# kupc25648/MOP-truss-MARL

Hardware: AMD Instinct MI355X
Metric: env steps/sec (batched FEM solves) at 4096 envs (higher is better)
Workload: dtype f64; 1 GPU; synthetic random-geometry 2-row trusses, 32 nodes / 80 elements / 60 DOF, FEM-only env.step (action decode + FP64 assembly/solve + stresses + point), no agent; envs_per_gpu=4096, global_envs=4096, nodes=32, elements=80, ndof=60, half_bandwidth=7, lanes_per_env=16, rows_per_lane=1, parallelism=env-batch sharded over 1 GPU(s), no data-path collective

## Files before the change

mop-truss-marl_amd/csrc/truss_body.h:

```cpp
#pragma once
#include <stdint.h>
#include <math.h>

#ifndef TB_SCHED_FENCE
#define TB_SCHED_FENCE()
#endif
#ifndef TRUSS_HD
#error "define TRUSS_HD (e.g. __device__ __forceinline__) before including truss_body.h"
#endif

#define TF_TOP 1
#define TF_RESX 2
#define TF_RESY 4
#define TF_LOAD_BRIDGE 8
#define TF_LOAD_ROOF 16

#define TB_NO_DECODE 0x1u
#define TB_CLAMP_INPLACE 0x2u
#define TB_EMIT_OBS 0x4u

#if defined(__clang__)
typedef uint32_t tb_u4 __attribute__((ext_vector_type(4)));
typedef uint32_t tb_u2 __attribute__((ext_vector_type(2)));
typedef float tb_f4 __attribute__((ext_vector_type(4)));
// ... 554 lines not shown
    }
  }

  TRUSS_HD void phase_assemble_nodes(const TopoDev &T) {
    const double *EV = evsh(T);
    const int16_t *AD = t_adj8(T), *DO = t_diagoff(T);
    double *K = kb(T);
    static_assert(NDEG == 8, "adjacency rows are read as one 16-byte unit");
    tb_u4 adj[NPL];
    int dof[NPL][3];
    double cc[NPL], cs[NPL], ss[NPL];
#pragma unroll
    for (int i = 0; i < NPL; ++i) {
      const int n0 = g + G * i, n = n0 < T.N ? n0 : T.N - 1;
      adj[i] = *(const tb_u4 *)(AD + n * NDEG);
      dof[i][0] = DO[3 * n];
      dof[i][1] = DO[3 * n + 1];
      dof[i][2] = DO[3 * n + 2];
      cc[i] = cs[i] = ss[i] = 0.0;
    }
#pragma unroll
    for (int h = 0; h < 2; ++h) {
      double ev[NPL][4][3];
#pragma unroll
      for (int i = 0; i < NPL; ++i)
#pragma unroll
        for (int a = 0; a < 4; ++a) {
          const uint32_t w = adj[i][2 * h + (a >> 1)];
          const int e = (a & 1) ? (int)(w >> 16) : (int)(w & 0xffffu);
          ev[i][a][0] = EV[3 * e + 0];
          ev[i][a][1] = EV[3 * e + 1];
          ev[i][a][2] = EV[3 * e + 2];
        }
#pragma unroll
      for (int i = 0; i < NPL; ++i)
#pragma unroll
        for (int a = 0; a < 4; ++a) {
          cc[i] += ev[i][a][0];
          cs[i] += ev[i][a][1];
          ss[i] += ev[i][a][2];
        }
    }
#pragma unroll
    for (int i = 0; i < NPL; ++i) {
      K[dof[i][0]] = cc[i];
      K[dof[i][1]] = ss[i];
      K[dof[i][2]] = cs[i];
    }
    for (int n = g + G * NPL; n < T.N; n += G) {
      double c2 = 0.0, s2 = 0.0, x2 = 0.0;
#pragma unroll
      for (int a = 0; a < NDEG; ++a) {
        const int e = AD[n * NDEG + a];
        c2 += EV[3 * e + 0];
        x2 += EV[3 * e + 1];
        s2 += EV[3 * e + 2];
      }
      K[DO[3 * n]] = c2;
      K[DO[3 * n + 1]] = s2;
      K[DO[3 * n + 2]] = x2;
    }
    const int idA = T.nteams == 1 ? T.ndof : T.ndof - T.KA;
    for (int r = idA + g; r < T.rowsA; r += G) K[r * W + r % W] = 1.0;
    for (int r = T.KA + T.mid + g; r < T.rowsB; r += G) K[(T.rowsA + r) * W + r % W] = 1.0;
  }

  TRUSS_HD void solver_scratch_init(const TopoDev &T) {
    double *Z = zs(T);
    const uint8_t *ZC = t_zcode(T);
    const int lbit = is_roof ? 4 : 2;
    {
      const int zt = T.zlen * T.nteams;
      constexpr int ZIT = 6;
#pragma unroll
      for (int i = 0; i < ZIT; ++i) {
        const int r0 = g + G * i, r = r0 < zt ? r0 : zt - 1;
        const int c = ZC[r];
        Z[r] = (c & lbit) ? ((c & 1) ? load_y : load_x) : 0.0;
      }
      for (int r = g + G * ZIT; r < zt; r += G) {
        const int c = ZC[r];
        Z[r] = (c & lbit) ? ((c & 1) ? load_y : load_x) : 0.0;
      }
    }
    tb_d2 *X2 = (tb_d2 *)__builtin_assume_aligned(xsol(T), 16);
    const tb_d2 z2 = {0.0, 0.0};
    for (int r = g; r < (T.zslot + 2) / 2; r += G) X2[r] = z2;
    double *RB = rbuf(T);
    for (int i = g; i < T.n_rest; i += G) RB[i] = 0.0;
  }

  TRUSS_HD void solver_init(const TopoDev &T) {
#pragma unroll
    for (int s = 0; s < RPL; ++s) {
      int r = gs + WL * s;
#pragma unroll
      for (int c = 0; c < W; ++c) R[s][c] = (c <= r) ? Kt[r * W + c] : Kt[c * W + r];
      rhs[s] = Zt[r];
    }
#pragma unroll
    for (int j = 0; j < W; ++j) xs[j] = 0.0;
  }

  double zkeep[RPL];
  TRUSS_HD void pivot_write(const TopoDev &T, int k, int kk) {
#pragma unroll
    for (int s = 0; s < RPL; ++s) Kt[k * W + gs + WL * s] = R[s][kk];
    bx = rhs[kk / WL];
  }
  TRUSS_HD void factor_z_store(const TopoDev &T, int kb, int c, int cnt) {
#pragma unroll
    for (int s = 0; s < RPL; ++s) {
      const int off = (gs + WL * s - c + W) % W;
      double *zp = off < cnt ? Zt + kb + off : ZRt + gs;
      *zp = zkeep[s];
    }
  }

  TRUSS_HD void pivot_update(const TopoDev &T, int k, int kk) {
    double col[W];
    {
      const double *Kn = Kt + (k + W) * W;
#pragma unroll
      for (int s = 0; s < RPL; ++s) ecol[s] = Kn[gs + WL * s];
    }
#pragma unroll
    for (int i = 0; i < W / 2; ++i) {
      tb_d2 v = ((const tb_d2 *)__builtin_assume_aligned(Kt + k * W, 16))[i];
      col[2 * i] = v[0];
      col[2 * i + 1] = v[1];
    }
    const double zk = tb_team_bcast(*this, kk % WL);
    if (gs == kk % WL) zkeep[kk / WL] = bx;
    const double d = col[kk];
    const double inv = tb_rcp(d);
#pragma unroll
    for (int s = 0; s < RPL; ++s) {
      double l = R[s][kk] * inv;
#pragma unroll
      for (int j = 0; j < W; ++j)
        if (j != kk) R[s][j] = fma(-l, col[j], R[s][j]);
      rhs[s] = fma(-l, zk, rhs[s]);
    }
#pragma unroll
    for (int s = 0; s < RPL; ++s) R[s][kk] = ecol[s];
    if (gs == kk % WL) {
      const int sp = kk / WL;
#pragma unroll
      for (int j = 0; j < W; ++j)
        if (j != kk) R[sp][j] = fr[sp][j];
      rhs[sp] = frhs[sp];
    }
  }
  double fr[RPL][W], frhs[RPL], ecol[RPL];
  TRUSS_HD void factor_rows_fetch(const TopoDev &T, int kb) {
#pragma unroll
    for (int s = 0; s < RPL; ++s) {
      const int rn = kb + W + gs + WL * s;
      const tb_d2 *K2 = (const tb_d2 *)__builtin_assume_aligned(Kt + rn * W, 16);
#pragma unroll
      for (int i = 0; i < W / 2; ++i) {
        tb_d2 v = K2[i];
        fr[s][2 * i] = v[0];
        fr[s][2 * i + 1] = v[1];
      }
      frhs[s] = Zt[rn];
    }
  }

  TRUSS_HD void pivot_check(const TopoDev &T) {
    const int lim = (T.nteams == 2 && team == 1) ? T.KA : (T.nteams == 2 ? T.KA + W : T.KA);
    for (int k = gs; k < lim; k += WL) {
      const double d = Kt[k * W + k % W];
      if (!(d > 0.0) || !(d < 1.7e308)) bad = 1;
    }
  }

  TRUSS_HD int win_row(const TopoDev &T, int slot) const { return T.KA + ((slot - T.KA % W + W) % W); }
  TRUSS_HD void merge_post(const TopoDev &T) {
    if (team == 1) {
      double *M = (double *)(L + T.o_mrg);
#pragma unroll
      for (int j = 0; j < W; ++j) M[gs * W + j] = R[0][j];
      M[W * W + gs] = rhs[0];
    }
  }
  TRUSS_HD void merge_take(const TopoDev &T) {
    if (team == 0) {
      const double *M = (const double *)(L + T.o_mrg);
      const int lim = T.ndof - T.KA;
      const int p = win_row(T, gs);
      const int pb = T.ndof - 1 - p;
#pragma unroll
      for (int j = 0; j < W; ++j) {
        const int c = win_row(T, j);
        const int cb = T.ndof - 1 - c;
        const bool ok = p < lim && c < lim;
        const double add = M[ok ? (pb % W) * W + (cb % W) : 0];
        R[0][j] += ok ? add : 0.0;
      }
      const double az = M[W * W + (p < lim ? pb % W : 0)];
      rhs[0] += p < lim ? az : 0.0;
    }
  }

  double bc[RPL][W], bz[RPL], bd[RPL];
  double nc[RPL][W], nz[RPL], nd[RPL];
  double bx;
  double myx[RPL] = {};
  TRUSS_HD void backsub_rows_fetch(const TopoDev &T, int kb) {
#pragma unroll
    for (int s = 0; s < RPL; ++s) {
      const int p = kb + gs + WL * s;
      const int pc = p < 0 ? 0 : p;
      const tb_d2 *K2 = (const tb_d2 *)__builtin_assume_aligned(Kt + pc * W, 16);
#pragma unroll
      for (int i = 0; i < W / 2; ++i) {
        tb_d2 v = K2[i];
        nc[s][2 * i] = v[0];
        nc[s][2 * i + 1] = v[1];
      }
      nz[s] = Zt[pc];
      nd[s] = Kt[pc * W + pc % W];
    }
  }
  TRUSS_HD void backsub_rows_adopt() {
#pragma unroll
    for (int s = 0; s < RPL; ++s) {
#pragma unroll
      for (int j = 0; j < W; ++j) bc[s][j] = nc[s][j];
      bz[s] = nz[s];
      bd[s] = tb_rcp(nd[s]);
    }
  }
  TRUSS_HD void backsub_step(const TopoDev &T, int k, int kk) {
    const int s = kk / WL;
    double acc0 = bz[s], acc1 = 0.0;
#pragma unroll
    for (int m = W - 1; m >= 2; --m) {
      const int j = (kk + m) % W;
      if (m & 1) acc1 = fma(-bc[s][j], xs[j], acc1);
      else acc0 = fma(-bc[s][j], xs[j], acc0);
    }
    const int jn = (kk + 1) % W;
    double acc = fma(-bc[s][jn], xs[jn], acc0 + acc1);
    bx = acc * bd[s];
  }
  TRUSS_HD void backsub_share(int kk) {
    xs[kk] = tb_team_bcast(*this, kk % WL);
    if (gs == kk % WL) myx[kk / WL] = bx;
  }
  TRUSS_HD bool owns_row(const TopoDev &T, int p) const {
    if (T.nteams == 1) return true;
    return team == 0 ? p < T.ndof - T.KA : p < T.KA;
  }
  TRUSS_HD void backsub_flush(const TopoDev &T, int kb) {
    double *XS = xsol(T);
#pragma unroll
    for (int s = 0; s < RPL; ++s) {
      const int p = kb + gs + WL * s;
      XS[owns_row(T, p) ? orig_pos(T, team, p) : T.zslot + 1] = myx[s];
    }
  }
  TRUSS_HD void backsub_flush_mid(const TopoDev &T) {
    double *XS = xsol(T);
    const int p = win_row(T, gs);
    XS[(team == 0 && owns_row(T, p)) ? p : T.zslot + 1] = myx[0];
  }
  TRUSS_HD void backsub_reload(const TopoDev &T) {
    const double *XS = xsol(T);
#pragma unroll
    for (int j = 0; j < W; ++j) {
      const int o = orig_pos(T, team, win_row(T, j));
      xs[j] = XS[(o >= 0 && o < T.ndof) ? o : T.zslot];
    }
  }

  TRUSS_HD float *oq0(const TopoDev &T) { return (float *)(L + T.o_kb + T.so_q0); }
  TRUSS_HD float *osr(const TopoDev &T) { return (float *)(L + T.o_kb + T.so_sr); }
  TRUSS_HD float *odisp(const TopoDev &T) { return (float *)(L + T.o_kb + T.so_disp); }
  TRUSS_HD float *omu(const TopoDev &T) { return (float *)(L + T.o_kb + T.so_mu); }
  TRUSS_HD float *omd(const TopoDev &T) { return (float *)(L + T.o_kb + T.so_md); }
  TRUSS_HD uint8_t *ocomp(const TopoDev &T) { return (uint8_t *)(L + T.o_kb + T.so_comp); }

  TRUSS_HD void phase_post_elements(const TopoDev &T, const StepArgsDev &A) {
    const double *XS = xsol(T);
    const int16_t *EX = t_exs(T);
    float *Q = oq0(T), *SR = osr(T);
    uint8_t *CP = ocomp(T);
    tb_u2 ex[EPL];
    double qv[EPL];
    float srv[EPL];
#pragma unroll
    for (int i = 0; i < EPL; ++i) {
      const int e = g + G * i;
      const int ee = e < T.E ? e : T.E - 1;
      ex[i] = *(const tb_u2 *)(EX + 4 * ee);
    }
    double v[EPL][4];
#pragma unroll
    for (int i = 0; i < EPL; ++i) {
      v[i][0] = XS[ex[i][0] & 0xffffu];
      v[i][1] = XS[ex[i][0] >> 16];
      v[i][2] = XS[ex[i][1] & 0xffffu];
      v[i][3] = XS[ex[i][1] >> 16];
    }
// ... 375 lines not shown
  TRUSS_HD void obs_nodes_raw(const TopoDev &T, const StepArgsDev &A) {
    if constexpr (EMIT) {
      load_params(T);
      float *Lf = (float *)L;
      const float *Y = ysh(T), *X = xsh(T), *TG = tgsh(T), *DS = odisp(T), *MU = omu(T), *MD = omd(T);
      const uint8_t *NFL = t_nflags(T);
      const float maxdef32 = (float)max_def;
      const int lbit = is_roof ? TF_LOAD_ROOF : TF_LOAD_BRIDGE;
#pragma unroll
      for (int c = 0; c < NDYN; ++c) {
        pmn[c] = INFINITY;
        pmx[c] = -INFINITY;
      }
#pragma unroll
      for (int i = 0; i < NPL; ++i) {
        const int n = g + G * i;
        const int nc = n < T.N ? n : T.N - 1;
        const int fl = NFL[nc];
        const float y = Y[nc];
        float *f = nfe[i];
        f[0] = X[nc];
        f[1] = y;
        f[2] = (fl & lbit) ? 1.0f : 0.0f;
        f[3] = MU[nc];
        f[4] = MD[nc];
        f[5] = (fl & TF_TOP) ? TG[nc] / (y + 1e-6f) : 0.0f;
        f[6] = fabsf(DS[2 * nc + 1]);
        const float ratio = f[6] / maxdef32;
        f[7] = fminf(ratio, 1.0f) * (ratio > 1.0f ? 1.0f : 0.5f);
        f[8] = ratio > 1.0f ? 1.0f : 0.0f;
        const tb_f4 raw = {f[2], f[5], f[6], ratio >= 1.0f ? 1.0f : 0.0f};
        ((tb_f4 *)(Lf + T.b_nraw))[nc] = raw;
        if (n < T.N) {
#pragma unroll
          for (int c = 0; c < NDYN; ++c) {
            pmn[c] = fminf(pmn[c], f[c]);
            pmx[c] = fmaxf(pmx[c], f[c]);
          }
        }
      }
    }
  }

  TRUSS_HD void obs_bank_fill(const TopoDev &T, const StepArgsDev &A) {
    if constexpr (EMIT) {
      float *Lf = (float *)L;
      float nv[NPL][NDYN];
#pragma unroll
      for (int c = 0; c < NDYN; ++c) {
        const float lo = tb_group_min(*this, c), hi = tb_group_max(*this, c);
        const float inv = tb_rcpf(hi - lo + 1e-6f);
#pragma unroll
        for (int i = 0; i < NPL; ++i) nv[i][c] = (nfe[i][c] - lo) * inv;
      }
#pragma unroll
      for (int i = 0; i < NPL; ++i) {
        const int n = g + G * i;
        const int nc = n < T.N ? n : T.N - 1;
        const tb_f4 a = {nv[i][0], nv[i][1], nv[i][2], nv[i][3]}, b = {nv[i][4], nv[i][5], nv[i][6], nv[i][7]};
        ((tb_f4 *)(Lf + T.b_nna))[nc] = a;
        ((tb_f4 *)(Lf + T.b_nnb))[nc] = b;
        Lf[T.b_nn8 + nc] = nv[i][8];
      }
    }
  }

  TRUSS_HD tb_f4 gather4(const float *Lf, const tb_u2 t) const {
    const tb_f4 v = {Lf[t[0] & 0xffffu], Lf[t[0] >> 16], Lf[t[1] & 0xffffu], Lf[t[1] >> 16]};
    return v;
  }
  template <int IT>
  TRUSS_HD void emit_rows(float *out, size_t row_floats, int nc, const tb_u2 (&tab)[IT]) const {
    if (!out) return;
    const float *Lf = (const float *)L;
    tb_f4 *o4 = (tb_f4 *)(out + (size_t)env * row_floats);
#pragma unroll
    for (int b0 = 0; b0 < IT; b0 += KB) {
      if (b0 * G < nc) {
        tb_f4 v[KB];
#pragma unroll
        for (int k = 0; k < KB; ++k)
          if (b0 + k < IT) v[k] = gather4(Lf, tab[b0 + k]);
#pragma unroll
        for (int k = 0; k < KB; ++k)
          if (b0 + k < IT) TB_OBS_STORE(&o4[chunk_of(b0 + k, nc)], v[k]);
      }
    }
  }
  TRUSS_HD void obs_nxe_table(const TopoDev &T) {
    if constexpr (EMIT) {
      if (T.nxe_cw != 4) return;
      const tb_u2 *tab = TB_TAB(tb_u2, TB, T.f_tnxe);
#pragma unroll
      for (int i = 0; i < IE; ++i) ete[i] = tab[i * G + g];
    }
  }
  TRUSS_HD void emit_nxe_narrow(const TopoDev &T, const StepArgsDev &A) const {
    if (!A.nxe) return;
    const float *Lf = (const float *)L;
    const uint16_t *tab = TB_TAB(uint16_t, TB, T.f_tnxe);
    float *o = A.nxe + (size_t)env * 21 * T.E;
    const int nc = T.nc_nxe;
    if (T.nxe_cw == 2) {
      for (int q0 = g; q0 < nc; q0 += 4 * G) {
        tb_f2 v[4];
#pragma unroll
        for (int k = 0; k < 4; ++k) {
          const int q = q0 + k * G < nc ? q0 + k * G : nc - 1;
          const tb_f2 w = {Lf[tab[2 * q]], Lf[tab[2 * q + 1]]};
          v[k] = w;
        }
#pragma unroll
        for (int k = 0; k < 4; ++k) {
          const int q = q0 + k * G < nc ? q0 + k * G : nc - 1;
          TB_OBS_STORE((tb_f2 *)o + q, v[k]);
        }
      }
    } else {
      for (int q0 = g; q0 < nc; q0 += 4 * G) {
        float v[4];
#pragma unroll
        for (int k = 0; k < 4; ++k) v[k] = Lf[tab[q0 + k * G < nc ? q0 + k * G : nc - 1]];
#pragma unroll
        for (int k = 0; k < 4; ++k) TB_OBS_STORE(o + (q0 + k * G < nc ? q0 + k * G : nc - 1), v[k]);
      }
    }
  }
  TRUSS_HD void obs_emit_raw_rows(const TopoDev &T, const StepArgsDev &A) {
    if constexpr (EMIT) {
      if (!active) return;
      if (T.nxe_cw == 4) emit_rows<IE>(A.nxe, (size_t)21 * T.E, T.nc_nxe, ete);
      else emit_nxe_narrow(T, A);
      emit_rows<IN_>(A.nxn, (size_t)12 * T.N, T.nc_nxn, etn);
    }
  }
  TRUSS_HD void obs_emit_xn(const TopoDev &T, const StepArgsDev &A) {
    if constexpr (EMIT) {
      if (!active) return;
      emit_rows<IX>(A.x_n, (size_t)13 * T.N, T.nc_xn, etx);
    }
  }
};

#ifndef TRUSS_ST
#define TRUSS_ST(i)
#endif
#define TRUSS_STREAM_SEG1(PH, T, A) PH(obs_emit_as(T, A));
#define TRUSS_STREAM_SEG2(PH, T, A) \
  PH(obs_emit_tc(T, A));            \
  PH(obs_nxe_table(T));
#define TRUSS_STREAM_SEG3(PH, T, A) \
  PH(obs_emit_raw_rows(T, A));      \
  PH(obs_emit_xn(T, A));
#define TRUSS_STEP_SCHEDULE(PH, PH_NS, BAR, T, A)                                   \
  TRUSS_ST(0);                                                                      \
  PH(phase_stage(T, A));                                                            \
  TRUSS_ST(1);                                                                      \
  PH(phase_decode(T, A));                                                           \
  if ((T).n_sym_nodes > 0 && !((A).flags & TB_NO_DECODE)) { PH(phase_sym_nodes(T)); } \
  TRUSS_ST(2);                                                                      \
  PH(phase_sizing(T, A));                                                           \
  if ((T).n_sym_elems > 0 && !((A).flags & TB_NO_DECODE)) { PH(phase_sym_elems(T)); } \
  if (EMIT_) { EMIT_POINT(1); TRUSS_ST(19); }  \
  PH_NS(rollout_prefetch(T, A));  \
  TRUSS_ST(3);                                                                      \
  PH(phase_elements(T, A));                                                         \
  TRUSS_ST(10);                                                                     \
  PH(phase_assemble_nodes(T));                                                      \
  TRUSS_ST(11);                                                                     \
  PH(solver_scratch_init(T));                                                       \
  TRUSS_ST(4);                                                                      \
  PH(solver_init(T));                                                               \
  {                                                                                 \
                                                                                    \
    const int kend_ = (T).nteams == 2 ? (T).KA + W_ : (T).KA;                       \
    int kb_ = 0;                                                                    \
    for (; kb_ + W_ <= (T).KA; kb_ += W_) {                                         \
      PH_NS(factor_rows_fetch(T, kb_));                                             \
      TRUSS_UNROLL                                                                  \
      for (int kk_ = 0; kk_ < W_; ++kk_) {                                          \
        PH(pivot_write(T, kb_ + kk_, kk_));                                         \
        PH_NS(pivot_update(T, kb_ + kk_, kk_));                                     \
      }                                                                             \
      PH_NS(factor_z_store(T, kb_, 0, W_));                                         \
    }                                                                               \
    TRUSS_ST(13);                                                                   \
                                  \
    if ((T).nteams == 2 && W_ <= 8) {                                               \
      const int c0_ = (T).KA % W_;                                                  \
      TRUSS_UNROLL                                                                  \
      for (int c_ = 0; c_ < W_; ++c_) {                                             \
        if (c_ == c0_) {                                                            \
          if (c_ > 0) { PH_NS(factor_rows_fetch(T, kb_)); }                         \
          TRUSS_UNROLL                                                              \
          for (int kk_ = 0; kk_ < c_; ++kk_) {                                      \
            PH(pivot_write(T, kb_ + kk_, kk_));                                     \
            PH_NS(pivot_update(T, kb_ + kk_, kk_));                                 \
          }                                                                         \
          if (c_ > 0) { PH_NS(factor_z_store(T, kb_, 0, c_)); }                     \
          PH(merge_post(T));                                                        \
          PH(merge_take(T));                                                        \
          TRUSS_UNROLL                                                              \
          for (int i_ = 0; i_ < W_; ++i_) {                                         \
            if ((c_ + i_) % W_ == 0) { PH_NS(factor_rows_fetch(T, (T).KA + i_)); }  \
            PH(pivot_write(T, (T).KA + i_, (c_ + i_) % W_));                        \
            PH_NS(pivot_update(T, (T).KA + i_, (c_ + i_) % W_));                    \
          }                                                                         \
          PH_NS(factor_z_store(T, (T).KA, c_, W_));                                 \
        }                                                                           \
      }                                                                             \
    } else if ((T).nteams == 2) {  \
      for (; kb_ < kend_; kb_ += W_) {                                              \
        PH_NS(factor_rows_fetch(T, kb_));                                           \
        TRUSS_UNROLL                                                                \
        for (int kk_ = 0; kk_ < W_; ++kk_) {                                        \
          if (kb_ + kk_ < kend_) {                                                  \
            if (kb_ + kk_ == (T).KA) {                                              \
              PH(merge_post(T));                                                    \
              PH(merge_take(T));                                                    \
            }                                                                       \
            PH(pivot_write(T, kb_ + kk_, kk_));                                     \
            PH_NS(pivot_update(T, kb_ + kk_, kk_));                                 \
          }                                                                         \
        }                                                                           \
        PH_NS(factor_z_store(T, kb_, 0, kend_ - kb_ < W_ ? kend_ - kb_ : W_));      \
      }                                                                             \
    }                                                                               \
    BAR();                                                                          \
    PH_NS(pivot_check(T));                                                          \
    TRUSS_ST(5);                                                                    \
                \
    kb_ = ((kend_ - 1) / W_) * W_;                                                  \
    PH_NS(backsub_rows_fetch(T, kb_));                                              \
    if ((T).nteams == 2 && W_ <= 8) {                                               \
      const int c0_ = (T).KA % W_;                                                  \
      TRUSS_UNROLL                                                                  \
      for (int c_ = 0; c_ < W_; ++c_) {                                             \
        if (c_ == c0_) {                                                            \
          PH_NS(backsub_rows_adopt());                                              \
          PH_NS(backsub_rows_fetch(T, kb_ - W_));                                   \
          TRUSS_UNROLL                                                              \
          for (int i_ = W_ - 1; i_ >= 0; --i_) {                                    \
            PH_NS(backsub_step(T, (T).KA + i_, (c_ + i_) % W_));                    \
            PH_NS(backsub_share((c_ + i_) % W_));                                   \
            if ((c_ + i_) % W_ == 0 && i_ > 0) {         \
              kb_ -= W_;                                                            \
              PH_NS(backsub_rows_adopt());                                          \
              PH_NS(backsub_rows_fetch(T, kb_ - W_));                               \
            }                                                                       \
          }                                                                         \
          PH_NS(backsub_flush_mid(T));                                              \
          BAR();                                                                    \
          PH_NS(backsub_reload(T));                                                 \
          TRUSS_UNROLL                                                              \
          for (int kk_ = c_ - 1; kk_ >= 0; --kk_) {                                 \
            PH_NS(backsub_step(T, kb_ + kk_, kk_));                                 \
            PH_NS(backsub_share(kk_));                                              \
          }                                                                         \
          if (c_ > 0) { PH_NS(backsub_flush(T, kb_)); }                             \
          kb_ -= W_;                                                                \
        }                                                                           \
      }                                                                             \
    } else if ((T).nteams == 2) {                                                   \
      for (; kb_ >= 0 && kb_ + W_ - 1 >= (T).KA - 1; kb_ -= W_) {                   \
        PH_NS(backsub_rows_adopt());                                                \
        PH_NS(backsub_rows_fetch(T, kb_ - W_));                                     \
        TRUSS_UNROLL                                                                \
        for (int kk_ = W_ - 1; kk_ >= 0; --kk_) {                                   \
          if (kb_ + kk_ < kend_) {                                                  \
            if (kb_ + kk_ == (T).KA - 1) {                                          \
              PH_NS(backsub_flush_mid(T));                                          \
              BAR();                                                                \
              PH_NS(backsub_reload(T));                                             \
            }                                                                       \
            PH_NS(backsub_step(T, kb_ + kk_, kk_));                                 \
            PH_NS(backsub_share(kk_));                                              \
          }                                                                         \
        }                                                                           \
        PH_NS(backsub_flush(T, kb_));                                               \
      }                                                                             \
    }                                                                               \
    TRUSS_ST(14);                                                                   \
    for (; kb_ >= 0; kb_ -= W_) {                                                   \
      PH_NS(backsub_rows_adopt());                                                  \
      PH_NS(backsub_rows_fetch(T, kb_ - W_));                                       \
      TRUSS_UNROLL                                                                  \
      for (int kk_ = W_ - 1; kk_ >= 0; --kk_) {                                     \
        PH_NS(backsub_step(T, kb_ + kk_, kk_));                                     \
        PH_NS(backsub_share(kk_));                                                  \
      }                                                                             \
      PH_NS(backsub_flush(T, kb_));                                                 \
    }                                                                               \
  }                                                                                 \
  BAR();                                                                            \
  TRUSS_ST(6);                                                                      \
  PH_NS(rollout_stash(T, A));                                                       \
  PH(phase_post_elements(T, A));                                                    \
  if (EMIT_) {                                                                      \
    EMIT_POINT(2);                                                                  \
    TRUSS_ST(18);                                                                   \
    PH(obs_elements_bank(T, A));                                                    \
  }                                                                                 \
  TRUSS_ST(7);                                                                      \
  PH(phase_post_nodes(T, A));                                                       \
  TRUSS_ST(8);                                                                      \
  if (EMIT_) {   \
    TRUSS_ST(15);                                                                   \
    PH(obs_nodes_raw(T, A));                                                        \
    TRUSS_ST(16);                                                                   \
    PH(obs_bank_fill(T, A));                                                        \
    EMIT_POINT(3);                                                                  \
    TRUSS_ST(17);                                                                   \
  }                                                                                 \
  PH_NS(phase_finish(T, A));                                                        \
  TRUSS_ST(12);                                                                     \
  PH_NS(phase_store(T, A));                                                         \
  TRUSS_ST(9);

struct ObsArgsDev {
  int32_t B;
  uint32_t flags;
  const float *x, *y;
  const int32_t *sec;
  const float *mu, *md, *target, *disp, *q0, *sr;
  const uint8_t *comp;
  const double *env_params;
  float *x_n, *A_s, *A_ts, *A_cs, *nxn, *nxe;
  int32_t tile_rows;
  int32_t n_split;
};

struct ObsLane {
  int lane, env;
  char *L;
  float maxdef32;
  int is_roof;
  int role;
  int minmax_done;

  TRUSS_HD float *raw() { return (float *)L; }
  TRUSS_HD float *mn(const TopoDev &T) { return raw() + T.N * 13; }
  TRUSS_HD float *mx(const TopoDev &T) { return mn(T) + 13; }
  TRUSS_HD float *part(const TopoDev &T) { return mx(T) + 13; }
  TRUSS_HD float *mats(const TopoDev &T) { return (float *)(L + (((size_t)(T.N * 13 + 26 + 128) * 4 + 15) & ~(size_t)15)); }

  TRUSS_HD void init(int lane_, int block, int tile, const TopoDev &, const ObsArgsDev &A, char *lds) {
    lane = lane_;
    env = block;
    L = lds;
    role = A.n_split <= 1 ? 0 : tile == 0 ? 2 : 1;
    minmax_done = 0;
    const double *P = A.env_params + (size_t)env * 8;
    maxdef32 = (float)P[2];
    is_roof = P[7] != 0.0;
  }

  TRUSS_HD void phase_nodes(const TopoDev &T, const ObsArgsDev &A) {
    if (role == 1) return;
    const size_t bn = (size_t)env * T.N;
// ... 182 lines not shown
```

mop-truss-marl_amd/csrc/truss_hip.hip:

```cpp
#include <hip/hip_runtime.h>

#include <atomic>
#include <cstdint>
#include <cstdio>
#include <cstring>
#include <type_traits>

#include "../../include/truss_mi355.h"

#pragma clang fp contract(off)

#define TRUSS_HD __device__ __forceinline__
#define TRUSS_UNROLL _Pragma("unroll")
#define TB_SCHED_FENCE() __builtin_amdgcn_sched_barrier(0)
#define TB_STREAM_STORE(p, v) __builtin_nontemporal_store((v), (p))
#ifdef TRUSS_OBS_STORE_NT
#define TB_OBS_STORE(p, v) __builtin_nontemporal_store((v), (p))
#else
#define TB_OBS_STORE(p, v) (*(p) = (v))
#endif

__device__ __forceinline__ void tb_lds_add(double *p, double v) { unsafeAtomicAdd(p, v); }

template <int WL, int SRC>
__device__ __forceinline__ double tb_dpp_bcast(double v) {
  const int lo = __double2loint(v), hi = __double2hiint(v);
  int rlo, rhi;
  if constexpr (WL == 16) {
    rlo = __builtin_amdgcn_update_dpp(lo, lo, 0x150 + SRC, 0xf, 0xf, false);
    rhi = __builtin_amdgcn_update_dpp(hi, hi, 0x150 + SRC, 0xf, 0xf, false);
  } else if constexpr (WL == 8) {
    rlo = __builtin_amdgcn_update_dpp(lo, lo, 0x150 + SRC, 0xf, 0x3, false);
    rlo = __builtin_amdgcn_update_dpp(rlo, lo, 0x150 + 8 + SRC, 0xf, 0xc, false);
    rhi = __builtin_amdgcn_update_dpp(hi, hi, 0x150 + SRC, 0xf, 0x3, false);
    rhi = __builtin_amdgcn_update_dpp(rhi, hi, 0x150 + 8 + SRC, 0xf, 0xc, false);
  } else {
    static_assert(WL == 4, "team width");
    constexpr int qp = SRC | (SRC << 2) | (SRC << 4) | (SRC << 6);
    rlo = __builtin_amdgcn_update_dpp(lo, lo, qp, 0xf, 0xf, false);
    rhi = __builtin_amdgcn_update_dpp(hi, hi, qp, 0xf, 0xf, false);
  }
  return __hiloint2double(rhi, rlo);
}
template <class LN>
__device__ __forceinline__ double tb_team_bcast(LN &ln, int src) {
  constexpr int WL = LN::WL_;
  switch (src) {
#define TB_CASE(i) \
  case i:          \
    if constexpr (i < WL) return tb_dpp_bcast<WL, i>(ln.bx); else break;
    TB_CASE(0) TB_CASE(1) TB_CASE(2) TB_CASE(3) TB_CASE(4) TB_CASE(5) TB_CASE(6) TB_CASE(7)
    TB_CASE(8) TB_CASE(9) TB_CASE(10) TB_CASE(11) TB_CASE(12) TB_CASE(13) TB_CASE(14) TB_CASE(15)
#undef TB_CASE
  }
  return ln.bx;
}

__device__ __forceinline__ double tb_rcp(double d) {
  double r = __builtin_amdgcn_rcp(d);
  r = fma(fma(-d, r, 1.0), r, r);
  r = fma(fma(-d, r, 1.0), r, r);
  return r;
}

__device__ __forceinline__ float tb_rcpf(float d) {
  float r = __builtin_amdgcn_rcpf(d);
  return fmaf(fmaf(-d, r, 1.0f), r, r);
}

#ifdef TRUSS_STOP_AT
#define TRUSS_ST(i) do { if ((i) == TRUSS_STOP_AT) return; } while (0)
#endif
#ifdef TRUSS_STAMPS
__device__ unsigned long long g_truss_stamps[32];
__device__ unsigned long long g_truss_span[4096][6];
#define TRUSS_ST(i)                                                  \
  do {                                                               \
    __builtin_amdgcn_sched_barrier(0);                               \
    if (threadIdx.x == 0 && blockIdx.x == gridDim.x / 2) g_truss_stamps[i] = clock64(); \
    if (threadIdx.x == 0 && ((i) == 0 || (i) == 9) && blockIdx.x < 4096) {              \
      g_truss_span[blockIdx.x][(i) == 0 ? 0 : 2] = clock64();                            \
      g_truss_span[blockIdx.x][(i) == 0 ? 1 : 3] = wall_clock64();                       \
    }                                                                \
    __builtin_amdgcn_sched_barrier(0);                               \
  } while (0)
#endif

__device__ __forceinline__ double tb_rsqrt(double x) {
  double r = __builtin_amdgcn_rsq(x);
  r = r * fma(-0.5 * x, r * r, 1.5);
  r = r * fma(-0.5 * x, r * r, 1.5);
  return r;
}

template <int G, bool MAX>
__device__ __forceinline__ float tb_group_reduce(float v) {
  auto op = [](float a, float b) { return MAX ? fmaxf(a, b) : fminf(a, b); };
  auto dpp = [](float x, auto ctrl) {
    return __int_as_float(__builtin_amdgcn_update_dpp(0, __float_as_int(x), decltype(ctrl)::value, 0xf, 0xf, false));
  };
  if constexpr (G >= 2) v = op(v, dpp(v, std::integral_constant<int, 0xB1>{}));
  if constexpr (G >= 4) v = op(v, dpp(v, std::integral_constant<int, 0x4E>{}));
  if constexpr (G >= 8) v = op(v, dpp(v, std::integral_constant<int, 0x141>{}));
  if constexpr (G >= 16) v = op(v, dpp(v, std::integral_constant<int, 0x140>{}));
  if constexpr (G >= 32) v = op(v, __shfl_xor(v, 16));
  if constexpr (G >= 64) v = op(v, __shfl_xor(v, 32));
  return v;
}
template <class LN>
__device__ __forceinline__ float tb_group_min(LN &ln, int c) { return tb_group_reduce<LN::G_, false>(ln.pmn[c]); }
template <class LN>
__device__ __forceinline__ float tb_group_max(LN &ln, int c) { return tb_group_reduce<LN::G_, true>(ln.pmx[c]); }

template <int G>
__device__ __forceinline__ double tb_group_reduce_sum(double v) {
  auto dpp = [](double x, auto ctrl) {
    const int lo = __builtin_amdgcn_update_dpp(0, __double2loint(x), decltype(ctrl)::value, 0xf, 0xf, false);
    const int hi = __builtin_amdgcn_update_dpp(0, __double2hiint(x), decltype(ctrl)::value, 0xf, 0xf, false);
    return __hiloint2double(hi, lo);
  };
  if constexpr (G >= 2) v = v + dpp(v, std::integral_constant<int, 0xB1>{});
  if constexpr (G >= 4) v = v + dpp(v, std::integral_constant<int, 0x4E>{});
  if constexpr (G >= 8) v = v + dpp(v, std::integral_constant<int, 0x141>{});
  if constexpr (G >= 16) v = v + dpp(v, std::integral_constant<int, 0x140>{});
  if constexpr (G >= 32) v = v + __shfl_xor(v, 16);
  if constexpr (G >= 64) v = v + __shfl_xor(v, 32);
  return v;
}
template <class LN>
__device__ __forceinline__ double tb_group_sum_d(LN &ln, int which) {
  return tb_group_reduce_sum<LN::G_>(which == 0 ? ln.p_vol : which == 1 ? ln.p_dt : ln.p_en);
}
template <class LN>
__device__ __forceinline__ float tb_group_max_f(LN &ln, int which) {
  return tb_group_reduce<LN::G_, true>(which == 0 ? ln.p_c1 : which == 1 ? ln.p_c2 : (float)ln.bad);
}

template <class LN, class TD>
__device__ __forceinline__ bool tb_obs_timed_out(LN &ln, const TD &T) {
  if constexpr (LN::EMIT_) return *((const __attribute__((address_space(3))) int *)(ln.TB + T.o_flag) + 1) != 0;
  return false;
}

#include "truss_body.h"

typedef __attribute__((address_space(3))) int tb_lds_word;
__device__ __forceinline__ tb_lds_word *tb_flag_ptr(char *lds, int o_flag) { return (tb_lds_word *)(lds + o_flag); }
__device__ __forceinline__ void tb_publish(char *lds, int o_flag, int k) {
  __builtin_amdgcn_wave_barrier();
#ifdef TRUSS_FLAG_RELAXED
  __builtin_amdgcn_fence(__ATOMIC_RELEASE, "wavefront");
  if (threadIdx.x == 0) __hip_atomic_store(tb_flag_ptr(lds, o_flag), k, __ATOMIC_RELAXED, __HIP_MEMORY_SCOPE_WORKGROUP);
#else
  if (threadIdx.x == 0) __hip_atomic_store(tb_flag_ptr(lds, o_flag), k, __ATOMIC_RELEASE, __HIP_MEMORY_SCOPE_WORKGROUP);
#endif
}
#ifndef TB_AWAIT_SPINS
#define TB_AWAIT_SPINS (1 << 22)
#endif
__device__ __forceinline__ bool tb_await(char *lds, int o_flag, int k) {
  for (int spin = 0; spin < TB_AWAIT_SPINS; ++spin) {
    const int v = __hip_atomic_load(tb_flag_ptr(lds, o_flag), __ATOMIC_ACQUIRE, __HIP_MEMORY_SCOPE_WORKGROUP);
    if (__builtin_amdgcn_readfirstlane(v) >= k) return true;
    __builtin_amdgcn_s_sleep(1);
  }
  return false;
}

template <class LN>
__device__ __forceinline__ void tb_obs_timeout(LN &ln, char *lds, int o_flag, int32_t *status) {
  if ((threadIdx.x & 63) == 0) *(tb_flag_ptr(lds, o_flag) + 1) = 1;
  if (ln.g == 0 && ln.active && status) atomicOr(&status[ln.env], TRUSS_STATUS_OBS_TIMEOUT);
}

template <int G, int WL, int RPL, int EPL, bool EMIT>
__global__ __launch_bounds__(EMIT ? 128 : 64) void truss_step_kernel(const TopoDev T, const StepArgsDev A) {
  extern __shared__ __attribute__((aligned(16))) char smem[];
  StepLane<G, WL, RPL, EPL, EMIT> ln;
  ln.init(threadIdx.x & 63, blockIdx.x, T, A, smem);
  constexpr int W_ = StepLane<G, WL, RPL, EPL, EMIT>::W;
  constexpr bool EMIT_ = EMIT;
  if constexpr (EMIT) {
    if (threadIdx.x == 0) {
      *tb_flag_ptr(smem, T.o_flag) = 0;
      *(tb_flag_ptr(smem, T.o_flag) + 1) = 0;
    }
    __syncthreads();
    if (threadIdx.x >= 64) {
#define SPH(call) \
  ln.call;        \
  __builtin_amdgcn_fence(__ATOMIC_RELEASE, "wavefront"); \
  __builtin_amdgcn_wave_barrier();                        \
  __builtin_amdgcn_fence(__ATOMIC_ACQUIRE, "wavefront")
#ifdef TRUSS_STAMPS
#define SST(i)                                                                                        \
  do {                                                                                                \
    __builtin_amdgcn_sched_barrier(0);                                                                \
    if (threadIdx.x == 64 && blockIdx.x == gridDim.x / 2) g_truss_stamps[i] = clock64();              \
    if (threadIdx.x == 64 && ((i) == 20 || (i) == 26) && blockIdx.x < 4096)                           \
      g_truss_span[blockIdx.x][(i) == 20 ? 4 : 5] = wall_clock64();                                   \
    __builtin_amdgcn_sched_barrier(0);                                                                \
  } while (0)
#else
#define SST(i)
#endif
      ln.emit_tables_load(T);
      __builtin_amdgcn_s_waitcnt(0);
      bool ok = tb_await(smem, T.o_flag, 1);
      if (ok) {
        SST(20);
        TRUSS_STREAM_SEG1(SPH, T, A)
        SST(21);
        ok = tb_await(smem, T.o_flag, 2);
      }
      if (ok) {
        SST(22);
        TRUSS_STREAM_SEG2(SPH, T, A)
        SST(23);
        ok = tb_await(smem, T.o_flag, 3);
      }
      if (ok) {
        SST(24);
        TRUSS_STREAM_SEG3(SPH, T, A)
        SST(25);
      } else {
        tb_obs_timeout(ln, smem, T.o_flag, A.status);
      }
#ifdef TRUSS_STAMPS
      __builtin_amdgcn_s_waitcnt(0);
      SST(26);
#endif
#undef SST
#undef SPH
      return;
    }
  }
#define TB_WAVE_SYNC()                                    \
  do {                                                    \
    __builtin_amdgcn_fence(__ATOMIC_RELEASE, "wavefront"); \
    __builtin_amdgcn_wave_barrier();                      \
    __builtin_amdgcn_fence(__ATOMIC_ACQUIRE, "wavefront"); \
  } while (0)
#define PH(call) \
  ln.call;       \
  TB_WAVE_SYNC()
#define PH_NS(call) ln.call
#define BAR() TB_WAVE_SYNC()
#ifdef TRUSS_FAULT_DROP_PUBLISH3
#define EMIT_POINT(k) do { if ((k) != 3) tb_publish(smem, T.o_flag, k); } while (0)
#else
#define EMIT_POINT(k) tb_publish(smem, T.o_flag, k)
#endif
  TRUSS_STEP_SCHEDULE(PH, PH_NS, BAR, T, A)
#undef PH
#undef PH_NS
#undef BAR
#undef EMIT_POINT
#undef TB_WAVE_SYNC
}

struct RolloutDev {
  TopoDev T;
  StepArgsDev A;
  int32_t n_steps, n_sets;
  size_t gstride, tstride;
};
template <int G, int WL, int RPL, int EPL>
__global__ __launch_bounds__(64) void truss_rollout_kernel(const RolloutDev P_) {
  extern __shared__ __attribute__((aligned(16))) char smem[];
  constexpr int W_ = StepLane<G, WL, RPL, EPL, false>::W;
  constexpr bool EMIT_ = false;
#define TB_WAVE_SYNC()                                    \
  do {                                                    \
    __builtin_amdgcn_fence(__ATOMIC_RELEASE, "wavefront"); \
    __builtin_amdgcn_wave_barrier();                      \
    __builtin_amdgcn_fence(__ATOMIC_ACQUIRE, "wavefront"); \
  } while (0)
#define PH(call) \
  ln.call;       \
  TB_WAVE_SYNC()
#define PH_NS(call) ln.call
#define BAR() TB_WAVE_SYNC()
#define EMIT_POINT(k) (void)0
  const int n_steps = P_.n_steps;
  for (int s = 0; s < n_steps; ++s) {
    typedef const char __attribute__((address_space(4))) *tb_kernarg_ptr;
    tb_kernarg_ptr ka = (tb_kernarg_ptr)__builtin_amdgcn_kernarg_segment_ptr();
    asm volatile("" : "+s"(ka));
    const RolloutDev &P = *(const RolloutDev *)ka;
    const TopoDev &T = P.T;
    const StepArgsDev &A = P.A;
    StepLane<G, WL, RPL, EPL, false> ln;
    ln.init(threadIdx.x, blockIdx.x, T, A, smem);
    const int nset = (s + 1) % P.n_sets;
    ln.rs_first_step = s;
    ln.rs_y_out = (s & 1) ? (float *)A.y_in : A.y_out;
    ln.rs_sec_out = (s & 1) ? (int32_t *)A.sec_in : A.sec_out;
    ln.rs_next_geo = s + 1 < n_steps ? A.a_geo + (size_t)nset * P.gstride : nullptr;
    ln.rs_next_topo = s + 1 < n_steps ? A.a_topo + (size_t)nset * P.tstride : nullptr;
    TRUSS_STEP_SCHEDULE(PH, PH_NS, BAR, T, A)
    TB_WAVE_SYNC();
  }
#undef PH
#undef PH_NS
#undef BAR
#undef EMIT_POINT
#undef TB_WAVE_SYNC
}

__global__ __launch_bounds__(64) void truss_obs_kernel(const TopoDev T, const ObsArgsDev A) {
  extern __shared__ __attribute__((aligned(16))) char smem[];
  ObsLane ln;
  ln.init(threadIdx.x, blockIdx.x, blockIdx.y, T, A, smem);
#define PH(call) \
  ln.call;       \
  __syncthreads()
#define PH_NS(call) ln.call
  const int r0_tile = ln.role == 1 ? ((int)blockIdx.y - 1) * A.tile_rows : 0;
  TRUSS_OBS_SCHEDULE(PH, PH_NS, T, A, r0_tile)
#undef PH
#undef PH_NS
}

__global__ __launch_bounds__(64) void truss_front_kernel(const truss_front_args_t A) {
  __shared__ double px[64], py[64], pc1[64], pc2[64];
  __shared__ double sx[64], sy[64], sd[64], scr[64];
  __shared__ int sidx[64], keep[64];
  __shared__ double ax[64], ay[64];
  const int b = blockIdx.x, i = threadIdx.x, P = A.max_points;
  int n = A.n_points[b];
  n = n < 0 ? 0 : (n > P ? P : n);
  const bool have = i < n;
  const double *row = A.points + ((size_t)b * P + (have ? i : 0)) * 4;
  const double x = row[0], y = row[1], c1 = row[2], c2 = row[3];
  px[i] = x; py[i] = y; pc1[i] = c1; pc2[i] = c2;
  __syncthreads();
  const bool feas = have && !(c1 > 1.0 || c2 > 1.0);
  bool dom = false, dup = false;
  for (int j = 0; j < n; ++j) {
    const bool fj = !(pc1[j] > 1.0 || pc2[j] > 1.0);
    dom |= fj && px[j] < x && py[j] < y;
    dup |= fj && j < i && px[j] == x && py[j] == y && pc1[j] == c1 && pc2[j] == c2;
  }
  const bool fr = feas && !dom && !dup;
  const double cx = fmin(x, 1.0), cy = fmin(y, 1.0);
  keep[i] = fr ? 1 : 0;
  __syncthreads();
  int rank = 0, arank = 0;
  for (int j = 0; j < n; ++j) {
    rank += keep[j] && (px[j] < x || (px[j] == x && (py[j] < y || (py[j] == y && j < i))));
    const double cxj = fmin(px[j], 1.0);
    arank += (cxj < cx || (cxj == cx && j < i));
  }
  __syncthreads();
  const unsigned long long fmask = __ballot(fr);
  int nf = __popcll(fmask);
  if (fr) { sx[rank] = x; sy[rank] = y; sidx[rank] = i; }
  if (have) { ax[arank] = cx; ay[arank] = cy; }
  __syncthreads();
  if (i + 1 < nf) {
    const double dx = sx[i] - sx[i + 1], dy = sy[i] - sy[i + 1];
    sd[i] = sqrt(dx * dx + dy * dy);
  }
  __syncthreads();
  if (i < nf) scr[i] = nf == 1 ? 0.0 : (i == 0 ? sd[0] : (i == nf - 1 ? sd[nf - 2] : sd[i - 1] + sd[i]));
  __syncthreads();
  bool kp = i < nf;
  if ((A.flags & TRUSS_FRONT_TRUNCATE) && nf > A.max_front) {
    if (i > 0 && i < nf - 1) {
      int cr = 0;
      for (int j = 1; j < nf - 1; ++j) cr += (scr[j] > scr[i] || (scr[j] == scr[i] && j < i));
      kp = cr < A.max_front - 2;
    }
  }
  const unsigned long long kmask = __ballot(kp);
  const int pos = __popcll(kmask & ((1ull << i) - 1ull));
  const int nk = __popcll(kmask);
  const double kx = i < nf ? sx[i] : 0.0, ky = i < nf ? sy[i] : 0.0;
  const int kid = i < nf ? sidx[i] : -1;
  __syncthreads();
  if (kp) { sx[pos] = kx; sy[pos] = ky; keep[pos] = kid; }
  nf = nk;
  __syncthreads();
  if (i + 1 < nf) {
    const double dx = sx[i] - sx[i + 1], dy = sy[i] - sy[i + 1];
    sd[i] = sqrt(dx * dx + dy * dy);
  }
  if (A.front_idx && i < P) A.front_idx[(size_t)b * P + i] = i < nf ? keep[i] : -1;
  __syncthreads();
  if (i != 0) return;
  if (A.n_front) A.n_front[b] = nf;
  const double rx = A.ref_points ? A.ref_points[2 * b] : 1.0, ry = A.ref_points ? A.ref_points[2 * b + 1] : 1.0;
  if (A.metrics) {
    double maxd = 0.0, disd = 1.0, sumd = 0.0, stdcd = 1.0, pn = 0.0;
    if (nf >= 2) {
      maxd = sd[0];
      for (int k = 0; k < nf - 1; ++k) { maxd = sd[k] > maxd ? sd[k] : maxd; sumd += sd[k]; }
      double acc = 0.0;
      const double ctr = maxd / (nf - 1);
      for (int k = 0; k < nf - 1; ++k) acc += (sd[k] - ctr) * (sd[k] - ctr);
      disd = sqrt(acc / (nf - 1));
    }
    if (nf > 3) {
      double s = 0.0, mx = 0.0;
      for (int k = 1; k < nf - 1; ++k) {
        const double cd = fabs(sx[k - 1] - sx[k + 1]) + fabs(sy[k - 1] - sy[k + 1]);
        scr[k] = cd; s += cd; mx = cd > mx ? cd : mx;
      }
      if (s != 0.0) {
        const int m = nf - 2;
        double mean = 0.0;
        for (int k = 1; k < nf - 1; ++k) { scr[k] = scr[k] / mx; mean += scr[k]; }
        mean /= m;
        double var = 0.0, p10 = 0.0;
        for (int k = 1; k < nf - 1; ++k) {
          const double v = scr[k], d = v - mean;
          var += d * d;
          const double v2 = v * v, v4 = v2 * v2;
          p10 += v4 * v4 * v2;
        }
        stdcd = sqrt(var / m);
        pn = pow(p10, 0.1);
      }
    }
// ... 556 lines not shown
```

Before: 225.8 million env-steps/s.

## Software-pipeline banded pivot steps so next pivot write overlaps current update

Splits each elimination pivot into a head, which updates the next pivot's column and the rhs, and a tail, which does the remaining row updates. The next pivot's write and diagonal read are issued between head and tail. This lets the wave-sync and LDS round-trip of the following pivot overlap with the trailing FMA work instead of serialising. It only applies to the non-emit, non-rollout kernel with team width of at least 8, and it adds register pressure from the extra pivot-column and multiplier arrays. The DPP broadcast also switches the first half-lane move from update_dpp to mov_dpp, which drops the old-value dependency.

```diff
diff --git a/mop-truss-marl_amd/csrc/truss_body.h b/mop-truss-marl_amd/csrc/truss_body.h
--- a/mop-truss-marl_amd/csrc/truss_body.h
+++ b/mop-truss-marl_amd/csrc/truss_body.h
@@ -730,6 +730,51 @@
       rhs[sp] = frhs[sp];
     }
   }
+  double pl[RPL], pcol[W], pd;
+  TRUSS_HD void pivot_lead_read(const TopoDev &T, int k, int kk) { pd = Kt[k * W + kk]; }
+  TRUSS_HD void pivot_head(const TopoDev &T, int k, int kk) {
+    const int kn = (kk + 1) % W;
+    {
+      const double *Kn = Kt + (k + W) * W;
+#pragma unroll
+      for (int s = 0; s < RPL; ++s) ecol[s] = Kn[gs + WL * s];
+    }
+#pragma unroll
+    for (int i = 0; i < W / 2; ++i) {
+      tb_d2 v = ((const tb_d2 *)__builtin_assume_aligned(Kt + k * W, 16))[i];
+      pcol[2 * i] = v[0];
+      pcol[2 * i + 1] = v[1];
+    }
+    const double zk = tb_team_bcast(*this, kk % WL);
+    if (gs == kk % WL) zkeep[kk / WL] = bx;
+    const double inv = tb_rcp(pd);
+#pragma unroll
+    for (int s = 0; s < RPL; ++s) {
+      pl[s] = R[s][kk] * inv;
+      R[s][kn] = fma(-pl[s], pcol[kn], R[s][kn]);
+      rhs[s] = fma(-pl[s], zk, rhs[s]);
+    }
+    if (gs == kk % WL) R[kk / WL][kn] = fr[kk / WL][kn];
+  }
+  TRUSS_HD void pivot_tail(const TopoDev &T, int k, int kk) {
+    TB_SCHED_FENCE();
+    const int kn = (kk + 1) % W;
+#pragma unroll
+    for (int s = 0; s < RPL; ++s) {
+#pragma unroll
+      for (int j = 0; j < W; ++j)
+        if (j != kk && j != kn) R[s][j] = fma(-pl[s], pcol[j], R[s][j]);
+    }
+#pragma unroll
+    for (int s = 0; s < RPL; ++s) R[s][kk] = ecol[s];
+    if (gs == kk % WL) {
+      const int sp = kk / WL;
+#pragma unroll
+      for (int j = 0; j < W; ++j)
+        if (j != kk && j != kn) R[sp][j] = fr[sp][j];
+      rhs[sp] = frhs[sp];
+    }
+  }
   double fr[RPL][W], frhs[RPL], ecol[RPL];
   TRUSS_HD void factor_rows_fetch(const TopoDev &T, int kb) {
 #pragma unroll
@@ -1411,6 +1456,23 @@
 #define TRUSS_STREAM_SEG3(PH, T, A) \
   PH(obs_emit_raw_rows(T, A));      \
   PH(obs_emit_xn(T, A));
+#ifndef TRUSS_PIVOT_PIPELINE
+#define TRUSS_PIVOT_PIPELINE 1
+#endif
+#define TRUSS_PIVOT_OPEN(PH, PH_NS, T, k, kk)  \
+  if (TRUSS_PIVOT_PIPELINE) {                  \
+    PH(pivot_write(T, k, kk));                 \
+    PH_NS(pivot_lead_read(T, k, kk));          \
+  }
+#define TRUSS_PIVOT(PH, PH_NS, T, k, kk, NEXT)                                 \
+  if (TRUSS_PIVOT_PIPELINE) {                                                  \
+    PH_NS(pivot_head(T, k, kk));                                               \
+    if (NEXT) { TRUSS_PIVOT_OPEN(PH, PH_NS, T, (k) + 1, ((kk) + 1) % W_) }     \
+    PH_NS(pivot_tail(T, k, kk));                                               \
+  } else {                                                                     \
+    PH(pivot_write(T, k, kk));                                                 \
+    PH_NS(pivot_update(T, k, kk));                                             \
+  }
 #define TRUSS_STEP_SCHEDULE(PH, PH_NS, BAR, T, A)                                   \
   TRUSS_ST(0);                                                                      \
   PH(phase_stage(T, A));                                                            \
@@ -1434,12 +1496,12 @@
                                                                                     \
     const int kend_ = (T).nteams == 2 ? (T).KA + W_ : (T).KA;                       \
     int kb_ = 0;                                                                    \
+    if (W_ <= (T).KA) { TRUSS_PIVOT_OPEN(PH, PH_NS, T, 0, 0) }                             \
     for (; kb_ + W_ <= (T).KA; kb_ += W_) {                                         \
       PH_NS(factor_rows_fetch(T, kb_));                                             \
       TRUSS_UNROLL                                                                  \
-      for (int kk_ = 0; kk_ < W_; ++kk_) {                                          \
-        PH(pivot_write(T, kb_ + kk_, kk_));                                         \
-        PH_NS(pivot_update(T, kb_ + kk_, kk_));                                     \
+      for (int kk_ = 0; kk_ < W_; ++kk_) {  \
+        TRUSS_PIVOT(PH, PH_NS, T, kb_ + kk_, kk_, kk_ + 1 < W_ || kb_ + 2 * W_ <= (T).KA); \
       }                                                                             \
       PH_NS(factor_z_store(T, kb_, 0, W_));                                         \
     }                                                                               \
@@ -1450,20 +1512,22 @@
       TRUSS_UNROLL                                                                  \
       for (int c_ = 0; c_ < W_; ++c_) {                                             \
         if (c_ == c0_) {                                                            \
-          if (c_ > 0) { PH_NS(factor_rows_fetch(T, kb_)); }                         \
+          if (c_ > 0) {                                                             \
+            PH_NS(factor_rows_fetch(T, kb_));                                       \
+            TRUSS_PIVOT_OPEN(PH, PH_NS, T, kb_, 0)                                         \
+          }                                                                         \
           TRUSS_UNROLL                                                              \
-          for (int kk_ = 0; kk_ < c_; ++kk_) {                                      \
-            PH(pivot_write(T, kb_ + kk_, kk_));                                     \
-            PH_NS(pivot_update(T, kb_ + kk_, kk_));                                 \
+          for (int kk_ = 0; kk_ < c_; ++kk_) {  \
+            TRUSS_PIVOT(PH, PH_NS, T, kb_ + kk_, kk_, kk_ + 1 < c_);                \
           }                                                                         \
           if (c_ > 0) { PH_NS(factor_z_store(T, kb_, 0, c_)); }                     \
           PH(merge_post(T));                                                        \
           PH(merge_take(T));                                                        \
+          TRUSS_PIVOT_OPEN(PH, PH_NS, T, (T).KA, c_)     \
           TRUSS_UNROLL                                                              \
           for (int i_ = 0; i_ < W_; ++i_) {                                         \
             if ((c_ + i_) % W_ == 0) { PH_NS(factor_rows_fetch(T, (T).KA + i_)); }  \
-            PH(pivot_write(T, (T).KA + i_, (c_ + i_) % W_));                        \
-            PH_NS(pivot_update(T, (T).KA + i_, (c_ + i_) % W_));                    \
+            TRUSS_PIVOT(PH, PH_NS, T, (T).KA + i_, (c_ + i_) % W_, i_ + 1 < W_);    \
           }                                                                         \
           PH_NS(factor_z_store(T, (T).KA, c_, W_));                                 \
         }                                                                           \
diff --git a/mop-truss-marl_amd/csrc/truss_hip.hip b/mop-truss-marl_amd/csrc/truss_hip.hip
--- a/mop-truss-marl_amd/csrc/truss_hip.hip
+++ b/mop-truss-marl_amd/csrc/truss_hip.hip
@@ -30,9 +30,9 @@
     rlo = __builtin_amdgcn_update_dpp(lo, lo, 0x150 + SRC, 0xf, 0xf, false);
     rhi = __builtin_amdgcn_update_dpp(hi, hi, 0x150 + SRC, 0xf, 0xf, false);
   } else if constexpr (WL == 8) {
-    rlo = __builtin_amdgcn_update_dpp(lo, lo, 0x150 + SRC, 0xf, 0x3, false);
+    rlo = __builtin_amdgcn_mov_dpp(lo, 0x150 + SRC, 0xf, 0x3, false);
     rlo = __builtin_amdgcn_update_dpp(rlo, lo, 0x150 + 8 + SRC, 0xf, 0xc, false);
-    rhi = __builtin_amdgcn_update_dpp(hi, hi, 0x150 + SRC, 0xf, 0x3, false);
+    rhi = __builtin_amdgcn_mov_dpp(hi, 0x150 + SRC, 0xf, 0x3, false);
     rhi = __builtin_amdgcn_update_dpp(rhi, hi, 0x150 + 8 + SRC, 0xf, 0xc, false);
   } else {
     static_assert(WL == 4, "team width");
@@ -142,6 +142,12 @@
   return false;
 }
 
+#ifndef TRUSS_PIVOT_PIPELINE
+#define TRUSS_PIVOT_PIPELINE PIPE_
+#endif
+template <int WL, bool EMIT, bool ROLLOUT>
+constexpr bool tb_pivot_pipeline() { return !EMIT && !ROLLOUT && WL >= 8; }
+
 #include "truss_body.h"
 
 typedef __attribute__((address_space(3))) int tb_lds_word;
@@ -180,6 +186,7 @@
   ln.init(threadIdx.x & 63, blockIdx.x, T, A, smem);
   constexpr int W_ = StepLane<G, WL, RPL, EPL, EMIT>::W;
   constexpr bool EMIT_ = EMIT;
+  [[maybe_unused]] constexpr bool PIPE_ = tb_pivot_pipeline<WL, EMIT, false>();
   if constexpr (EMIT) {
     if (threadIdx.x == 0) {
       *tb_flag_ptr(smem, T.o_flag) = 0;
@@ -270,6 +277,7 @@
   extern __shared__ __attribute__((aligned(16))) char smem[];
   constexpr int W_ = StepLane<G, WL, RPL, EPL, false>::W;
   constexpr bool EMIT_ = false;
+  [[maybe_unused]] constexpr bool PIPE_ = tb_pivot_pipeline<WL, false, true>();
 #define TB_WAVE_SYNC()                                    \
   do {                                                    \
     __builtin_amdgcn_fence(__ATOMIC_RELEASE, "wavefront"); \
```

Result: slower. 217.4 million env-steps/s (-3.7%).
